# albertgassol1/vf-nerf

Hardware: AMD Instinct MI355X
Metric: rays/sec (4096-ray chunk, 128 samples/ray) + PSNR vs ref (higher is better)
Workload: dtype f16x3+f32acc

## Files before the change

### vf_nerf_amd/csrc/vfn_mlp16.hip

```cpp
#include <string.h>
#include <utility>
#include "vfn_common.h"
#include "vfn_plan.h"

typedef _Float16 half8 __attribute__((ext_vector_type(8)));
typedef _Float16 half2v __attribute__((ext_vector_type(2)));
typedef float float2v __attribute__((ext_vector_type(2)));
typedef float f32x16 __attribute__((ext_vector_type(16)));
typedef float f32x4v __attribute__((ext_vector_type(4)));

#ifndef VFN16_ASCALE
#define VFN16_ASCALE 1
#endif
#define VFN16_WSCALE 64.0f
#define VFN16_INV_WSCALE 0.015625f
#define VFN16_PACK_WSCALE (VFN16_ASCALE ? 1.0f : VFN16_WSCALE)
#define VFN16_XSCALE (VFN16_ASCALE ? VFN16_WSCALE : 1.0f)
#ifndef VFN16_SAVE_AUX
#define VFN16_SAVE_AUX 2
#endif
#ifndef VFN16_HANDOVER_NUM
#define VFN16_HANDOVER_NUM 8
#endif
#ifndef VFN16_DMA_STEPS
// ... 248 lines not shown
constexpr ChunkD chunk_of(int mode, int c) {
    if (!(mode & M16_BLKIN)) {
        const int vf_layers = (mode & M16_FEAT) ? 9 : 8;
        for (int h = 0; h < vf_layers; ++h) {
            if (c < VF_TILES[h]) return {0, vf_off_kb(h) + c * chunk_kb(VF_ACT[h], VF_AUX[h]), chunk_kb(VF_ACT[h], VF_AUX[h]), VF_AUX[h]};
            c -= VF_TILES[h];
        }
        if (c == 0) return {0, vf_off_kb(9), HEAD_KB, 0};
        c -= 1;
    }
    if (mode & M16_RENDER) {
        for (int h = 0; h < 4; ++h) {
            if (c < RN_TILES[h]) return {1, rn_off_kb(h) + c * chunk_kb(RN_ACT[h], RN_AUX[h]), chunk_kb(RN_ACT[h], RN_AUX[h]), RN_AUX[h]};
            c -= RN_TILES[h];
        }
        if (c == 0) return {1, rn_off_kb(4), HEAD_KB, 0};
    }
    return {0, 0, 0, 0};
}

constexpr int rn_first_chunk(int mode) { return (mode & M16_BLKIN) ? 0 : 72; }
constexpr bool chunk_two(int mode, int c) { return (mode & M16_C2) && !(mode & M16_BLKIN) && c >= 63 && c != 71; }
constexpr bool mode_one(int mode) { return (mode & M16_P1) != 0; }
#ifndef VFN16_P1_RING
#define VFN16_P1_RING 5
#endif
#define VFN16_P1_SLOT_KB 20
constexpr int ring_of(int mode) { return mode_one(mode) ? VFN16_P1_RING : 3; }
constexpr int slot_u4(int mode) { return mode_one(mode) ? VFN16_P1_SLOT_KB * 64 : VFN16_MAX_CHUNK_KB * 64; }
constexpr int slot_base(int mode, int c) { return (c % ring_of(mode)) * slot_u4(mode); }
static_assert(VFN16_P1_RING * VFN16_P1_SLOT_KB <= 3 * VFN16_MAX_CHUNK_KB, "the single-product ring must fit into the split modes' ring");
constexpr int stores_of(int mode, int c) { return (c == 0 || ((mode & M16_RENDER) && c == rn_first_chunk(mode))) ? 0 : 4; }
constexpr int young_ops(int mode, int c) {
    const int ring = ring_of(mode);
    int n = 0;
    for (int k = (c - ring + 2 > 0 ? c - ring + 2 : 0); k < c; ++k) n += stores_of(mode, k);
    for (int j = 2; j <= ring - 2; ++j)
        if (c + j >= ring - 1 && chunk_of(mode, c + j).kb > 0) n += (((chunk_of(mode, c + j).kb - 1) / 2 + 1) / VFN16_WAVES);
    return n;
}

struct Mlp16Args {
    const uint4* vf_w;
    const uint4* rn_w;
    const float* points;
    const float* ray_dirs;
    float* out_vec;
    float* out_colors;
    long long n_points;
    int dirs_div;
    int vf_multires, rn_multires;
    uint32_t vf_bytes, rn_bytes;
    float* saved;
    float* save_aux_vf;
// ... 17 lines not shown
#define VFN16_RANGE_TRACK 2
#endif

struct X16 { half8 hi[16]; half8 lo[16]; };
struct A16 { half8 hi[3]; half8 lo[3]; };

struct Pipe16 {
    uint4* lds;
    __amdgpu_buffer_rsrc_t vf_w;
    __amdgpu_buffer_rsrc_t rn_w;
    float* saved;
    long long slot_floats;
    uint32_t slot_bytes;
    uint32_t save_voff;
    uint32_t save_voff16;
    uint32_t feat_voff;
    uint32_t st_tile, st_q;
    int save16;
    uint32_t* masks;
    uint32_t mask_bytes;
    uint32_t mask_voff;
    uint4* blk_out;
    uint32_t blk_bytes, blk_voff;
};

struct Carry16 {
    f32x16 pend;
    f32x16 bias;
    half8 fh0, fl0;
    uint32_t lm[4];
    unsigned long long sat;
};

template <int N, typename F, int... I>
__device__ __forceinline__ void static_for_impl(F&& f, std::integer_sequence<int, I...>) { (f(std::integral_constant<int, I>{}), ...); }
template <int N, typename F>
__device__ __forceinline__ void static_for(F&& f) { static_for_impl<N>(f, std::make_integer_sequence<int, N>{}); }

__device__ __forceinline__ void split2(float a, float b, _Float16& h0, _Float16& h1, _Float16& l0, _Float16& l1) {
    const float2v v = {a, b};
    const half2v hi = __builtin_convertvector(v, half2v);
    h0 = hi[0]; h1 = hi[1];
    const uint32_t hp = __builtin_bit_cast(uint32_t, hi);
    float r0, r1;
    asm("v_fma_mix_f32 %0, %1, -1.0, %2 op_sel_hi:[1,0,0]" : "=v"(r0) : "v"(hp), "v"(a));
    asm("v_fma_mix_f32 %0, %1, -1.0, %2 op_sel:[1,0,0] op_sel_hi:[1,0,0]" : "=v"(r1) : "v"(hp), "v"(b));
    const float2v r = {r0, r1};
    const half2v lo = __builtin_convertvector(r, half2v);
    l0 = lo[0]; l1 = lo[1];
}

__device__ __forceinline__ float tanh_exp(float v) { return 1.0f - 2.0f / (1.0f + expf(2.0f * v)); }

template <int NET, int OFF_KB, int LDS_U4>
__device__ __forceinline__ void dma_piece(const Pipe16& p, int blk, int lane, int dst_blk = -1) {
    __builtin_amdgcn_raw_ptr_buffer_load_lds(NET ? p.rn_w : p.vf_w, (lds_void*)(p.lds + LDS_U4 + (dst_blk < 0 ? blk : dst_blk) * 64), 16,
                                             lane * 16, (OFF_KB + blk) * 1024, 0, 0);
}
template <int MODE, int C>
__device__ __forceinline__ void dma_chunk(const Pipe16& p, int wave, int lane) {
    constexpr ChunkD d = chunk_of(MODE, C);
    if constexpr (mode_one(MODE)) {
        constexpr int NKB = (d.kb - 1) / 2;
#pragma unroll
        for (int i = 0; i * VFN16_WAVES < NKB + 1; ++i)
            if (wave + VFN16_WAVES * i < NKB + 1) dma_piece<d.net, d.off_kb, slot_base(MODE, C)>(p, 2 * (wave + VFN16_WAVES * i), lane, wave + VFN16_WAVES * i);
    } else {
#pragma unroll
    for (int i = 0; i * VFN16_WAVES < d.kb; ++i)
        if (wave + VFN16_WAVES * i < d.kb) dma_piece<d.net, d.off_kb, slot_base(MODE, C)>(p, wave + VFN16_WAVES * i, lane);
    }
}

template <int MODE, int C>
__device__ __forceinline__ void prefetch_chunk(Carry16& cy, const Pipe16& p, int lane) {
    constexpr ChunkD d = chunk_of(MODE, C);
    const uint4* cb = p.lds + slot_base(MODE, C);
    const f32x4v* bb = reinterpret_cast<const f32x4v*>(cb + (mode_one(MODE) ? (d.kb - 1) / 2 : d.kb - 1) * 64) + (lane >> 5) * 4;
    const f32x4v b0 = bb[0], b1 = bb[1], b2 = bb[2], b3 = bb[3];
#pragma unroll
    for (int q = 0; q < 4; ++q) { cy.bias[q] = b0[q]; cy.bias[4 + q] = b1[q]; cy.bias[8 + q] = b2[q]; cy.bias[12 + q] = b3[q]; }
    cy.fh0 = __builtin_bit_cast(half8, cb[0 * 64 + lane]);
    if (!chunk_two(MODE, C) && !mode_one(MODE)) cy.fl0 = __builtin_bit_cast(half8, cb[1 * 64 + lane]);
}

template <int EPI, bool KEEP, bool LO = true>
__device__ __forceinline__ void epi_pair(f32x16& pend, unsigned long long& sat, int pr, half8& hi, half8& lo, int j) {
    float v0 = pend[2 * pr], v1 = pend[2 * pr + 1];
#if VFN16_RANGE_TRACK == 1
    if (EPI == EPI_RELU) sat |= __builtin_amdgcn_ballot_w64(fmaxf(v0, v1) >= VFN16_CLAMP);
#endif
    if (!VFN16_ASCALE || EPI != EPI_RELU) { v0 *= VFN16_INV_WSCALE; v1 *= VFN16_INV_WSCALE; }
    if (EPI == EPI_RELU) {
        v0 = fminf(fmaxf(v0, 0.f), VFN16_CLAMP); v1 = fminf(fmaxf(v1, 0.f), VFN16_CLAMP);
    }
    else { v0 = tanh_exp(v0) * VFN16_XSCALE; v1 = tanh_exp(v1) * VFN16_XSCALE; }
    if constexpr (LO) {
        _Float16 h0, h1, l0, l1;
        split2(v0, v1, h0, h1, l0, l1);
        hi[j] = h0; hi[j + 1] = h1; lo[j] = l0; lo[j + 1] = l1;
// ... 85 lines not shown

template <int MODE, int C0, int ACT, int AUX, int NCH, int EPI, int PEPI, int PKB, int SLOT = -1, int PSLOT = -1, bool BLK = false,
          bool PBLK = false>
__device__ __forceinline__ void layer16(const X16& xin, const A16& aux, X16& xout, X16& xpend, Carry16& cy, float (&head)[3],
                                       const Pipe16& p, int wave, int lane) {
    constexpr int NKB = ACT + AUX;
    constexpr int E = NKB / 2 > 0 ? NKB / 2 : 1;
    constexpr int H = NKB * VFN16_HANDOVER_NUM / 16 > 0 ? NKB * VFN16_HANDOVER_NUM / 16 : 1;
    constexpr int PMAX = (VFN16_MAX_CHUNK_KB + VFN16_WAVES - 1) / VFN16_WAVES;
    constexpr int DSPAN = NKB - H > 0 ? NKB - H : 1;
    constexpr int DSTEPS = DSPAN < VFN16_DMA_STEPS ? DSPAN : VFN16_DMA_STEPS;
    static_assert(PEPI < 0 || PKB >= E, "the pending tile must be complete before it is read");
    constexpr bool TRAIN = (MODE & M16_TRAIN) != 0;
    constexpr bool LATE = TRAIN && VFN16_LATE_STORES;
    constexpr int DEND = LATE ? (NKB - 4 > H + 1 ? NKB - 4 : (H + 1 < NKB ? H + 1 : NKB - 1)) : 0;
    constexpr int SBEG = LATE ? DEND : H;
    constexpr int SSTEPS = LATE ? (NKB - DEND > 0 ? NKB - DEND : 1) : (DSPAN < 4 ? DSPAN : 4);
    constexpr int DST = LATE ? (DEND - H > 0 ? DEND - H : 1) : DSTEPS;
    constexpr int MPARTS = (LATE && E <= H) ? (DEND - H >= 4 ? 4 : (DEND - H >= 2 ? 2 : (DEND - H >= 1 ? 1 : 0))) : 0;
    static_for<NCH>([&](auto ich) {
        constexpr int ch = decltype(ich)::value;
        constexpr int C = C0 + ch;
        constexpr int RING = ring_of(MODE);
        constexpr ChunkD dcur = chunk_of(MODE, C), dnext = chunk_of(MODE, C + 1), ddma = chunk_of(MODE, C + RING - 1);
        static_assert(dcur.kb == 2 * NKB + 1, "layer shape and chunk table disagree");
        constexpr bool P1 = mode_one(MODE);
        constexpr bool W2 = chunk_two(MODE, C);
        constexpr bool D2 = chunk_two(MODE, C + RING - 1) || P1;
        constexpr int DNKB = (ddma.kb - 1) / 2;
        constexpr int DPIECES = P1 ? DNKB + 1 : (D2 ? DNKB + ddma.aux + 1 : ddma.kb);
        auto piece_blk = [&](int idx) -> int {
            if (P1) return idx < DNKB ? 2 * idx : 2 * DNKB;
            if (!D2) return idx;
            if (ddma.aux == 0) return 2 * idx;
            return idx < DNKB ? 2 * idx : (idx < DNKB + ddma.aux ? 2 * (idx - ddma.aux) + 1 : 2 * DNKB);
        };
        constexpr int PM = D2 ? (DPIECES + VFN16_WAVES - 1) / VFN16_WAVES : PMAX;
        const uint4* cb = p.lds + slot_base(MODE, C);
        constexpr int FB = P1 ? 1 : 2;
        f32x16 acc = cy.bias;
        half8 fh[VFN16_FDEPTH], fl[VFN16_FDEPTH];
        fh[0] = cy.fh0;
        if (!P1 && (!W2 || ACT == 0)) fl[0] = cy.fl0;
        if (VFN16_FDEPTH == 3 && NKB > 1) {
            fh[1] = __builtin_bit_cast(half8, cb[FB * 64 + lane]);
            if (!W2 && !P1) fl[1] = __builtin_bit_cast(half8, cb[3 * 64 + lane]);
        }
        half8 ehi[2], elo[2];
        [[maybe_unused]] unsigned mbits = 0;
#pragma unroll
        for (int st = 0; st < NKB; ++st) {
            constexpr int AHEAD = VFN16_FDEPTH - 1;
            if (st + AHEAD < NKB) {
                fh[(st + AHEAD) % VFN16_FDEPTH] = __builtin_bit_cast(half8, cb[(FB * (st + AHEAD)) * 64 + lane]);
                if (!P1 && (!W2 || st + AHEAD >= ACT)) fl[(st + AHEAD) % VFN16_FDEPTH] = __builtin_bit_cast(half8, cb[(2 * (st + AHEAD) + 1) * 64 + lane]);
            }
            const half8 a_hi = fh[st % VFN16_FDEPTH];
            const half8 x_hi = st < ACT ? xin.hi[st < ACT ? st : 0] : aux.hi[st >= ACT ? st - ACT : 0];
            const half8 x_lo = st < ACT ? xin.lo[st < ACT ? st : 0] : aux.lo[st >= ACT ? st - ACT : 0];
            acc = __builtin_amdgcn_mfma_f32_32x32x16_f16(a_hi, x_hi, acc, 0, 0, 0);
#ifndef ABL_P1
// ... 14 lines not shown
                    if (ch > 0) epi_pair<EPI, TRAIN, !P1>(cy.pend, cy.sat, pr, ehi[sblk], elo[sblk], j);
                    else epi_pair<(PEPI >= 0 ? PEPI : 0), TRAIN, !P1>(cy.pend, cy.sat, pr, ehi[sblk], elo[sblk], j);
                    if ((pr & 3) == 3) {
                        asm volatile("" : "+a"(ehi[sblk]));
                        if constexpr (!P1) asm volatile("" : "+a"(elo[sblk]));
                        if (ch > 0) { xout.hi[2 * (ch > 0 ? ch - 1 : 0) + sblk] = ehi[sblk]; if constexpr (!P1) xout.lo[2 * (ch > 0 ? ch - 1 : 0) + sblk] = elo[sblk]; }
                        else { xpend.hi[PKB + sblk] = ehi[sblk]; if constexpr (!P1) xpend.lo[PKB + sblk] = elo[sblk]; }
                    }
                }
#ifndef VFN16_NOGROUPS
                if constexpr (!P1) {
                __builtin_amdgcn_sched_group_barrier(0x100, W2 ? 1 : 2, 0);
                __builtin_amdgcn_sched_group_barrier(0x008, 1, 0);
                __builtin_amdgcn_sched_group_barrier(0x002, W2 ? VFN16_EPI_PER_MFMA2 : VFN16_EPI_PER_MFMA, 0);
                __builtin_amdgcn_sched_group_barrier(0x008, 1, 0);
                __builtin_amdgcn_sched_group_barrier(0x002, W2 ? VFN16_EPI_PER_MFMA2 : VFN16_EPI_PER_MFMA, 0);
                if (!W2) {
                    __builtin_amdgcn_sched_group_barrier(0x008, 1, 0);
                    __builtin_amdgcn_sched_group_barrier(0x002, VFN16_EPI_PER_MFMA, 0);
                }
                }
#endif
            }
            if (st == H - 1 && dnext.kb > 0) {
#ifndef ABL_NOSYNC
#ifdef ABL_LOOSE_WAIT
                if ((MODE & M16_TRAIN) != 0) asm volatile("s_waitcnt vmcnt(4)" ::: "memory");
                else
#endif
                if constexpr (P1 && LATE) {
                    constexpr int young = young_ops(MODE, C);
                    static_assert(young < 64, "vmcnt is a 6-bit field");
                    if constexpr (young == 0) asm volatile("s_waitcnt vmcnt(0)" ::: "memory");
                    else asm volatile("s_waitcnt vmcnt(%0)" :: "n"(young) : "memory");
                } else
                if (LATE && C > 0 && (ch == 0 || ch > 1 || PEPI >= 0)) asm volatile("s_waitcnt vmcnt(4)" ::: "memory");
                else asm volatile("s_waitcnt vmcnt(0)" ::: "memory");
                __builtin_amdgcn_s_barrier();
#endif
            }
#ifndef ABL_NODMA
            if (st >= H && st < H + DST && ddma.kb > 0) {
#pragma unroll
                for (int i = (st - H) * PM / DST; i < (st - H + 1) * PM / DST; ++i) {
                    if (VFN16_WAVES * i + VFN16_WAVES <= DPIECES) dma_piece<ddma.net, ddma.off_kb, slot_base(MODE, C + RING - 1)>(p, piece_blk(wave + VFN16_WAVES * i), lane, P1 ? wave + VFN16_WAVES * i : -1);
                    else if (VFN16_WAVES * i < DPIECES) {
                        const int idx = min(wave + VFN16_WAVES * i, DPIECES - 1);
                        dma_piece<ddma.net, ddma.off_kb, slot_base(MODE, C + RING - 1)>(p, piece_blk(idx), lane, P1 ? idx : -1);
                    }
                }
            }
#endif
#ifndef ABL_NOMASK
            if (TRAIN && MPARTS > 0 && st >= H && st < H + MPARTS && (ch > 0 || PEPI >= 0)) {
                static_for<MPARTS>([&](auto ip) {
                    constexpr int part = decltype(ip)::value;
                    if (st - H == part) {
                        if (ch > 0) collect_mask_part<(ch > 0 ? ch - 1 : 0), EPI, part, (MPARTS > 0 ? MPARTS : 1)>(cy, mbits);
                        else collect_mask_part<PKB / 2, (PEPI >= 0 ? PEPI : 0), part, (MPARTS > 0 ? MPARTS : 1)>(cy, mbits);
                    }
                });
            }
#endif
            if (TRAIN && st >= SBEG && st < SBEG + SSTEPS && (ch > 0 || PEPI >= 0)) {
#ifndef ABL_NOMASK
                if (st == (LATE ? SBEG : VFN16_MASK_STEP(H, NKB))) {
                    if constexpr (MPARTS > 0) {
                        if (ch == 0) store_mask<(PSLOT >= 0 ? PSLOT : 0)>(p, cy);
                    } else {
                        if (ch > 0) collect_mask<(ch > 0 ? ch - 1 : 0), EPI>(cy);
                        else { collect_mask<PKB / 2, (PEPI >= 0 ? PEPI : 0)>(cy); store_mask<(PSLOT >= 0 ? PSLOT : 0)>(p, cy); }
                    }
                }
#endif
#pragma unroll
                for (int q = (st - SBEG) * 4 / SSTEPS; q < (st - SBEG + 1) * 4 / SSTEPS; ++q) {
                    if (ch > 0) save_group<(SLOT >= 0 ? SLOT : 0), (ch > 0 ? ch - 1 : 0), (MODE & M16_SF16) != 0>(p, cy.pend, q);
                    else save_group<(PSLOT >= 0 ? PSLOT : 0), PKB / 2, (MODE & M16_SF16) != 0>(p, cy.pend, q);
                }
            }
            if (st == H && ((BLK && ch > 0) || (PBLK && ch == 0))) {
                if (ch > 0) store_blocks<(ch > 0 ? ch - 1 : 0)>(p, xout);
                else store_blocks<PKB / 2>(p, xpend);
            }
            if (st == NKB - 1 && dnext.kb > 0) prefetch_chunk<MODE, (dnext.kb > 0 ? C + 1 : C)>(cy, p, lane);
#ifndef VFN16_NOSCHED
            __builtin_amdgcn_sched_barrier(0);
#endif
        }
        if (EPI == EPI_RELU || EPI == EPI_TANH) {
            cy.pend = acc;
#if VFN16_RANGE_TRACK == 2
            if (EPI == EPI_RELU) {
                float mx = fmaxf(acc[0], acc[1]);
#pragma unroll
                for (int r = 2; r < 16; r += 2) mx = fmaxf(mx, fmaxf(acc[r], acc[r + 1]));
                cy.sat |= __builtin_amdgcn_ballot_w64(mx >= VFN16_CLAMP);
            }
#endif
        } else {
#pragma unroll
            for (int c = 0; c < 3; ++c) {
                const float v = acc[c] * VFN16_INV_WSCALE;
                head[c] = (EPI == EPI_HEAD_TANH) ? tanh_exp(v) : 1.0f / (1.0f + expf(-v));
            }
        }
    });
}
// ... 91 lines not shown
    layer16<MODE, C0 + 16, 16, 0, 8, R, R, 14, 11, 10>(xb, aux, xa, xb, cy, rgb, p, wave, lane);
    layer16<MODE, C0 + 24, 16, 0, 8, R, R, 14, 12, 11>(xa, aux, xb, xa, cy, rgb, p, wave, lane);
    layer16<MODE, C0 + 32, 16, 0, 1, EPI_HEAD_SIGMOID, R, 14, -1, 12>(xb, aux, xa, xb, cy, rgb, p, wave, lane);
    const long long mo = m;
    if (in && (threadIdx.x & 32) == 0) {
        a.out_vec[mo * 3 + 0] = nrm[0]; a.out_vec[mo * 3 + 1] = nrm[1]; a.out_vec[mo * 3 + 2] = nrm[2];
        a.out_colors[mo * 3 + 0] = rgb[0]; a.out_colors[mo * 3 + 1] = rgb[1]; a.out_colors[mo * 3 + 2] = rgb[2];
    }
}

__device__ __forceinline__ void report_range(const Mlp16Args& a, unsigned long long sat, float ain) {
    if (a.status) {
        const unsigned bits = (sat != 0ull ? 1u : 0u) | (ain >= VFN16_CLAMP ? 2u : 0u);
        if (bits) atomicOr(a.status, bits);
    }
}

template <int MODE>
__global__ __launch_bounds__(256, 1) void vfn_mlp16_kernel(const Mlp16Args a) {
    __shared__ __attribute__((aligned(16))) uint4 s_ring[3 * VFN16_SLOT + 256 * 8];
    float* s_park = reinterpret_cast<float*>(s_ring + 3 * VFN16_SLOT) + threadIdx.x * 32;
    const int tid = threadIdx.x;
    const int lane = tid & 63;
    const int wave = __builtin_amdgcn_readfirstlane(tid >> 6);
    const int g = lane >> 5;
#ifdef VFN16_STAMPS
    const unsigned long long st_t0 = __builtin_amdgcn_s_memtime(), st_r0 = __builtin_amdgcn_s_memrealtime();
#endif
    unsigned long long ck_t0 = 0ull, ck_r0 = 0ull;
    if constexpr ((MODE & M16_RENDER) != 0 && (MODE & M16_BLKIN) == 0 && (MODE & M16_TRAIN) == 0) {
        if (a.clock) { ck_t0 = __builtin_amdgcn_s_memtime(); ck_r0 = __builtin_amdgcn_s_memrealtime(); }
    }
    const long long m = (long long)blockIdx.x * VFN16_PTS + wave * 32 + (lane & 31);
    long long n_live = a.n_points;
    if (a.n_dev) {
        const long long nd = (long long)*a.n_dev;
        n_live = nd < n_live ? nd : n_live;
        if ((long long)blockIdx.x * VFN16_PTS >= n_live) return;
    }
    const bool in = m < n_live;

    if constexpr ((MODE & M16_BLKIN) != 0) {
        const int dpos = in ? a.src[m] : -1;
        const bool live = dpos >= 0;
        float xr[3] = {0.f, 0.f, 0.f}, dr[3] = {0.f, 0.f, 0.f}, nrm[3] = {0.f, 0.f, 0.f};
        if (live) {
            const long long di = dpos / a.dirs_div;
#pragma unroll
            for (int c = 0; c < 3; ++c) { xr[c] = a.points[(long long)dpos * 3 + c]; dr[c] = a.ray_dirs[di * 3 + c]; nrm[c] = a.vec_in[m * 3 + c]; }
        }
        Pipe16 p;
        p.lds = s_ring;
        p.vf_w = __builtin_amdgcn_make_buffer_rsrc(const_cast<uint4*>(a.rn_w), 0, (int)a.rn_bytes, 0x00020000);
        p.rn_w = p.vf_w;
        p.saved = nullptr; p.slot_floats = 0; p.slot_bytes = 0; p.save_voff = 0; p.blk_out = nullptr; p.blk_bytes = 0; p.blk_voff = 0;
        p.masks = nullptr; p.mask_bytes = 0; p.mask_voff = 0; p.save16 = 0; p.save_voff16 = 0; p.feat_voff = 0; p.st_tile = 0; p.st_q = 0;
        dma_chunk<MODE, 0>(p, wave, lane);
        dma_chunk<MODE, 1>(p, wave, lane);
        X16 xa, xb;
        A16 aux;
        float ain_blk = 0.f;
        {
            typedef unsigned int u32x4 __attribute__((ext_vector_type(4)));
            const __amdgpu_buffer_rsrc_t rs_blk = __builtin_amdgcn_make_buffer_rsrc(
                const_cast<uint4*>(a.blk_in), 0, (int)(((a.n_points + 31) & ~31ll) * 1024), 0x00020000);
            const unsigned goff = in ? (unsigned)((m >> 5) * 32768 + lane * 16) : 0xfffffff0u;
            u32x4 q[32];
#pragma unroll
            for (int i = 0; i < 32; ++i) q[i] = __builtin_amdgcn_raw_buffer_load_b128(rs_blk, goff, i * 1024, 0);
            render_aux<MODE>(a, aux, xr, dr, nrm, -1, false, g, ain_blk);
#pragma unroll
            for (int t = 0; t < 8; ++t) {
                half8 h0 = __builtin_bit_cast(half8, q[4 * t + 0]), l0 = __builtin_bit_cast(half8, q[4 * t + 1]);
                half8 h1 = __builtin_bit_cast(half8, q[4 * t + 2]), l1 = __builtin_bit_cast(half8, q[4 * t + 3]);
                asm volatile("" : "+a"(h0)); asm volatile("" : "+a"(l0)); asm volatile("" : "+a"(h1)); asm volatile("" : "+a"(l1));
                xb.hi[2 * t] = h0; xb.lo[2 * t] = l0; xb.hi[2 * t + 1] = h1; xb.lo[2 * t + 1] = l1;
            }
        }
        asm volatile("s_waitcnt vmcnt(0)" ::: "memory");
        __builtin_amdgcn_s_barrier();
        Carry16 cy;
#pragma unroll
        for (int q = 0; q < 16; ++q) cy.pend[q] = 0.f;
        cy.lm[0] = 0; cy.lm[1] = 0; cy.lm[2] = 0; cy.lm[3] = 0; cy.sat = 0ull;
        prefetch_chunk<MODE, 0>(cy, p, lane);
#ifdef VFN16_STAMPS
        const unsigned long long st_t1 = __builtin_amdgcn_s_memtime();
#endif
        render_tail<MODE>(a, p, cy, xa, xb, aux, nrm, live ? (long long)dpos : -1, live, wave, lane);
        report_range(a, cy.sat, ain_blk);
#ifdef VFN16_STAMPS
        if (threadIdx.x == 0 && live) {
            const unsigned long long t2 = __builtin_amdgcn_s_memtime(), r2 = __builtin_amdgcn_s_memrealtime();
            a.out_colors[(long long)dpos * 3 + 0] = (float)(st_t1 - st_t0); a.out_colors[(long long)dpos * 3 + 1] = (float)(t2 - st_t0);
            a.out_colors[(long long)dpos * 3 + 2] = (float)(r2 - st_r0);
        }
#endif
    } else {
    float x[3] = {0.f, 0.f, 0.f};
    if (in) { x[0] = a.points[m * 3 + 0]; x[1] = a.points[m * 3 + 1]; x[2] = a.points[m * 3 + 2]; }
    float d[3] = {0.f, 0.f, 0.f};
    int out_row = -1;
    if ((MODE & M16_RENDER) && in) {
        const long long di = m / a.dirs_div;
        d[0] = a.ray_dirs[di * 3 + 0]; d[1] = a.ray_dirs[di * 3 + 1]; d[2] = a.ray_dirs[di * 3 + 2];
        if (a.out_index) out_row = a.out_index[m];
    }
    asm volatile("s_waitcnt vmcnt(0)" ::: "memory");
    if (MODE & M16_RENDER) {
        s_park[0] = x[0]; s_park[1] = x[1]; s_park[2] = x[2];
        s_park[4] = d[0]; s_park[5] = d[1]; s_park[6] = d[2];
    }

    Pipe16 p;
    p.lds = s_ring;
    p.vf_w = __builtin_amdgcn_make_buffer_rsrc(const_cast<uint4*>(a.vf_w), 0, (int)a.vf_bytes, 0x00020000);
    p.rn_w = __builtin_amdgcn_make_buffer_rsrc(const_cast<uint4*>((MODE & M16_RENDER) ? a.rn_w : a.vf_w), 0,
                                               (int)((MODE & M16_RENDER) ? a.rn_bytes : a.vf_bytes), 0x00020000);
    const bool frag = (a.save_f16 & 2) != 0;
    const long long mw = m + a.ws_first;
    p.slot_floats = frag ? ((a.ws_points + 31) >> 5) * 8192 : a.ws_points * 256;
    p.saved = a.saved + a.ws_first * 256;
    {
        const long long left = p.slot_floats * 4 - a.ws_first * 1024;
        p.slot_bytes = (uint32_t)(left < 0x7fffffffll ? left : 0x7fffffffll);
    }
    p.save_voff = !in ? (frag ? 0xc0000000u : 0xfffffff0u) : (frag ? (uint32_t)((m >> 5) * 32768 + lane * 16) : (uint32_t)(m * 1024 + g * 16));
    p.save_voff16 = !in ? (frag ? 0xc0000000u : 0xfffffff0u) : (frag ? (uint32_t)((m >> 5) * 32768 + lane * 8) : (uint32_t)(m * 1024 + g * 8));
    p.feat_voff = in ? (uint32_t)(m * 1024 + g * 16) : 0xfffffff0u;
    p.st_tile = frag ? 4096u : 128u; p.st_q = frag ? 1024u : 32u;
    p.masks = a.save_masks; p.mask_bytes = (uint32_t)(a.ws_points * 32); p.mask_voff = in ? (uint32_t)((2 * mw + g) * 16) : 0xfffffff0u;
    p.save16 = a.save_f16 & 1;
    p.blk_out = a.blk_out; p.blk_bytes = (uint32_t)(((a.n_points + 31) & ~31ll) * 1024);
    p.blk_voff = (uint32_t)((m >> 5) * 32768 + lane * 16);
    dma_chunk<MODE, 0>(p, wave, lane);
    dma_chunk<MODE, 1>(p, wave, lane);
    if constexpr (mode_one(MODE)) static_for<VFN16_P1_RING - 3>([&](auto ic) { dma_chunk<MODE, 2 + decltype(ic)::value>(p, wave, lane); });
#ifdef ABL_NODMA
    dma_chunk<MODE, 9>(p, wave, lane);
    dma_chunk<MODE, 10>(p, wave, lane);
    dma_chunk<MODE, 11>(p, wave, lane);
#endif

    const int vf_multires = a.vf_multires;
    A16 aux;
    float ain = 0.f;
    {
        float sn[18], cs[18];
        encode_sincos(x, vf_multires, g, sn, cs);
        build_aux(aux, g, [&](int k) { return enc_value(x, sn, cs, vf_multires, k); }, ain);
        if ((MODE & M16_TRAIN) && in) save_aux(a.save_aux_vf, mw, g, [&](int k) { return enc_value(x, sn, cs, vf_multires, k); });
        half8* pk = reinterpret_cast<half8*>(s_park + 8);
#pragma unroll
        for (int q = 0; q < 3; ++q) { pk[2 * q] = aux.hi[q]; pk[2 * q + 1] = aux.lo[q]; }
    }
    asm volatile("s_waitcnt vmcnt(0)" ::: "memory");
    __builtin_amdgcn_s_barrier();
    Carry16 cy;
#pragma unroll
    for (int q = 0; q < 16; ++q) cy.pend[q] = 0.f;
    cy.lm[0] = 0; cy.lm[1] = 0; cy.lm[2] = 0; cy.lm[3] = 0; cy.sat = 0ull;
    prefetch_chunk<MODE, 0>(cy, p, lane);

    X16 xa, xb;
    float vec[3] = {0.f, 0.f, 0.f};
#ifdef VFN16_STAMPS
    const unsigned long long st_t1 = __builtin_amdgcn_s_memtime();
#endif
    constexpr int R = EPI_RELU, T = EPI_TANH, NONE = -1;
    layer16<MODE, 0, 0, 3, 8, R, NONE, 0, 0, -1>(xa, aux, xb, xb, cy, vec, p, wave, lane);
    layer16<MODE, 8, 16, 0, 8, R, R, 14, 1, 0>(xb, aux, xa, xb, cy, vec, p, wave, lane);
    layer16<MODE, 16, 16, 0, 8, R, R, 14, 2, 1>(xa, aux, xb, xa, cy, vec, p, wave, lane);
    layer16<MODE, 24, 16, 0, 7, R, R, 14, 3, 2>(xb, aux, xa, xb, cy, vec, p, wave, lane);
    { A16 ax; load_aux(ax, s_park); layer16<MODE, 31, 14, 3, 8, R, R, 12, 4, 3>(xa, ax, xb, xa, cy, vec, p, wave, lane); }
    layer16<MODE, 39, 16, 0, 8, R, R, 14, 5, 4>(xb, aux, xa, xb, cy, vec, p, wave, lane);
    layer16<MODE, 47, 16, 0, 8, R, R, 14, 6, 5>(xa, aux, xb, xa, cy, vec, p, wave, lane);
    layer16<MODE, 55, 16, 0, 8, R, R, 14, 7, 6>(xb, aux, xa, xb, cy, vec, p, wave, lane);
    if constexpr (!(MODE & M16_FEAT)) {
        layer16<MODE, 63, 16, 0, 1, EPI_HEAD_TANH, R, 14, -1, 7>(xa, aux, xb, xa, cy, vec, p, wave, lane);
        if (in && g == 0) { a.out_vec[m * 3 + 0] = vec[0]; a.out_vec[m * 3 + 1] = vec[1]; a.out_vec[m * 3 + 2] = vec[2]; }
        report_range(a, cy.sat, ain);
    } else {
    constexpr bool BO = (MODE & M16_BLKOUT) != 0;
    layer16<MODE, 63, 16, 0, 8, T, R, 14, 8, 7, BO, false>(xa, aux, xb, xa, cy, vec, p, wave, lane);
    layer16<MODE, 71, 16, 0, 1, EPI_HEAD_TANH, T, 14, -1, 8, false, BO>(xa, aux, xb, xb, cy, vec, p, wave, lane);
    if constexpr (!(MODE & M16_RENDER)) {
        if (in && g == 0) { a.out_vec[m * 3 + 0] = vec[0]; a.out_vec[m * 3 + 1] = vec[1]; a.out_vec[m * 3 + 2] = vec[2]; }
        report_range(a, cy.sat, ain);
#ifdef VFN16_STAMPS
        if (threadIdx.x == 0) {
            const unsigned long long t2 = __builtin_amdgcn_s_memtime(), r2 = __builtin_amdgcn_s_memrealtime();
            a.out_vec[m * 3 + 0] = (float)(st_t1 - st_t0); a.out_vec[m * 3 + 1] = (float)(t2 - st_t0); a.out_vec[m * 3 + 2] = (float)(r2 - st_r0);
        }
#endif
    } else {
    float nrm[3];
#pragma unroll
    for (int c = 0; c < 3; ++c) nrm[c] = __shfl(vec[c], lane & 31, 64);
    const float xr[3] = {s_park[0], s_park[1], s_park[2]};
    const float dr[3] = {s_park[4], s_park[5], s_park[6]};
    A16 raux;
    render_aux<MODE>(a, raux, xr, dr, nrm, (MODE & M16_TRAIN) ? mw : m, in, g, ain);
    render_tail<MODE>(a, p, cy, xa, xb, raux, nrm, a.out_index ? (long long)out_row : m, a.out_index ? out_row >= 0 : in, wave, lane);
    report_range(a, cy.sat, ain);
    if constexpr ((MODE & M16_TRAIN) == 0) {
        if (a.clock && threadIdx.x == 0 && (long long)blockIdx.x < a.clock_slots) {
            const unsigned long long t1 = __builtin_amdgcn_s_memtime(), r1 = __builtin_amdgcn_s_memrealtime();
            a.clock[2 * blockIdx.x] = t1 - ck_t0; a.clock[2 * blockIdx.x + 1] = r1 - ck_r0;
        }
    }
    const long long mo = (long long)blockIdx.x * VFN16_PTS + (threadIdx.x >> 6) * 32 + (threadIdx.x & 31);
    (void)mo;
#ifdef VFN16_STAMPS
    if (threadIdx.x == 0) {
        const unsigned long long t1 = __builtin_amdgcn_s_memtime(), r1 = __builtin_amdgcn_s_memrealtime();
        a.out_colors[mo * 3 + 0] = (float)(t1 - st_t0); a.out_colors[mo * 3 + 1] = (float)(r1 - st_r0);
    }
#endif
    }
    }
    }
}

int check_vf16(const Plan16& vf, const char* what) {
    bool ok = vf.feat_layer == 1 && vf.n_hidden == 9 && (int)vf.head_off_kb == vf_off_kb(9);
    for (int h = 0; ok && h < 9; ++h)
        ok = vf.act16[h] == VF_ACT[h] && vf.aux16[h] == VF_AUX[h] && vf.n_tiles[h] == VF_TILES[h] && (int)vf.off_kb[h] == vf_off_kb(h);
    if (!ok) { vfn_set_error("%s: the f16x3 kernels are specialised for the shipped vector-field network shape", what); return VFN_ERR_UNSUPPORTED; }
    return VFN_OK;
}
int check_rn16(const Plan16& rn, const char* what) {
    bool ok = rn.n_hidden == 4 && (int)rn.head_off_kb == rn_off_kb(4);
    for (int h = 0; ok && h < 4; ++h)
        ok = rn.act16[h] == RN_ACT[h] && rn.aux16[h] == RN_AUX[h] && rn.n_tiles[h] == RN_TILES[h] && (int)rn.off_kb[h] == rn_off_kb(h);
    if (!ok) { vfn_set_error("%s: the f16x3 kernels are specialised for the shipped rendering network shape", what); return VFN_ERR_UNSUPPORTED; }
    return VFN_OK;
}

}

static int check_kind16(int net_kind, const Plan16& p, const char* what) {
    return net_kind == VFN_NET_VF ? check_vf16(p, what) : check_rn16(p, what);
// ... 22 lines not shown
    : old_status(t_status_word), old_clock(t_clock_probe), old_slots(t_clock_slots) {
    if (status_word) t_status_word = status_word;
    if (clock_stamps && clock_slots > 0) { t_clock_probe = reinterpret_cast<unsigned long long*>(clock_stamps); t_clock_slots = clock_slots; }
}
VfnReportScope::~VfnReportScope() { t_status_word = old_status; t_clock_probe = old_clock; t_clock_slots = old_slots; }

extern "C" int vfn_vf_mlp16_fwd(const vfn_net_geom* geom, const void* packed16, const float* points, int64_t n_points,
                                 float* out_vec, void* stream) {
    Mlp16Args a = {};
    VfnNetPlan p32; Plan16 vf;
    int rc = make_plan16(VFN_NET_VF, geom, &p32, &vf, "vfn_vf_mlp16_fwd");
    if (rc != VFN_OK) return rc;
    rc = check_vf16(vf, "vfn_vf_mlp16_fwd");
    if (rc != VFN_OK) return rc;
    if (n_points <= 0) return VFN_OK;
    VFN_REQUIRE(packed16 && points && out_vec, "vfn_vf_mlp16_fwd: NULL argument");
    a.vf_w = (const uint4*)packed16; a.points = points; a.out_vec = out_vec; a.n_points = n_points; a.dirs_div = 1;
    a.vf_multires = vf.multires; a.vf_bytes = vf.total_kb * 1024u;
    a.status = t_status_word;
    a.clock = t_clock_probe; a.clock_slots = t_clock_slots;
    const long long blocks = (n_points + VFN16_PTS - 1) / VFN16_PTS;
    hipLaunchKernelGGL(vfn_mlp16_kernel<M16_VF_VEC>, dim3((unsigned)blocks), dim3(256), 0, (hipStream_t)stream, a);
    return vfn_check_launch("vfn_vf_mlp16_fwd");
}

static int launch_fused16(const char* what, const vfn_net_geom* vf_geom, const void* vf_packed16, const vfn_net_geom* rn_geom,
                          const void* rn_packed16, const float* points, const float* ray_dirs, int64_t n_points,
                          int32_t samples_per_ray, const int32_t* out_index, bool scatter, int32_t colour_products, float* normals,
                          float* colors, void* stream, const int32_t* n_dev = nullptr) {
    Mlp16Args a = {};
    a.n_dev = n_dev;
    VfnNetPlan p32; Plan16 vf, rn;
    VFN_REQUIRE(vf_geom && rn_geom, "%s: NULL argument", what);
    int rc = make_plan16(VFN_NET_VF, vf_geom, &p32, &vf, what);
    if (rc != VFN_OK) return rc;
    rc = make_plan16(VFN_NET_RENDER, rn_geom, &p32, &rn, what);
    if (rc != VFN_OK) return rc;
    rc = check_vf16(vf, what);
    if (rc != VFN_OK) return rc;
    rc = check_rn16(rn, what);
    if (rc != VFN_OK) return rc;
    VFN_REQUIRE(vf_geom->feature_dims == VFN_HIDDEN && rn_geom->feature_dims == VFN_HIDDEN, "%s: both nets need feature_dims == %d", what, VFN_HIDDEN);
    VFN_REQUIRE(colour_products == 2 || colour_products == 3, "%s: colour_products must be 2 or 3 (got %d)", what, colour_products);
    if (n_points <= 0) return VFN_OK;
    VFN_REQUIRE(vf_packed16 && rn_packed16 && points && ray_dirs && normals && colors && (out_index || !scatter), "%s: NULL argument", what);
    VFN_REQUIRE(samples_per_ray > 0, "%s: samples_per_ray must be > 0", what);
    a.vf_w = (const uint4*)vf_packed16; a.rn_w = (const uint4*)rn_packed16; a.points = points; a.ray_dirs = ray_dirs;
    a.out_vec = normals; a.out_colors = colors; a.out_index = out_index; a.n_points = n_points; a.dirs_div = samples_per_ray;
    a.vf_multires = vf.multires; a.rn_multires = rn.multires; a.vf_bytes = vf.total_kb * 1024u; a.rn_bytes = rn.total_kb * 1024u;
    a.status = t_status_word;
    a.clock = t_clock_probe; a.clock_slots = t_clock_slots;
    const long long blocks = (n_points + VFN16_PTS - 1) / VFN16_PTS;
    if (colour_products == 2) hipLaunchKernelGGL(vfn_mlp16_kernel<M16_FUSED | M16_C2>, dim3((unsigned)blocks), dim3(256), 0, (hipStream_t)stream, a);
    else hipLaunchKernelGGL(vfn_mlp16_kernel<M16_FUSED>, dim3((unsigned)blocks), dim3(256), 0, (hipStream_t)stream, a);
    return vfn_check_launch(what);
}

extern "C" int vfn_vf_render_fused16_fwd(const vfn_net_geom* vf_geom, const void* vf_packed16, const vfn_net_geom* rn_geom,
                                          const void* rn_packed16, const float* points, const float* ray_dirs,
                                          int64_t n_points, int32_t samples_per_ray, float* normals, float* colors,
                                          void* stream) {
    return launch_fused16("vfn_vf_render_fused16_fwd", vf_geom, vf_packed16, rn_geom, rn_packed16, points, ray_dirs, n_points, samples_per_ray,
                          nullptr, false, 3, normals, colors, stream);
}

extern "C" int vfn_vf_render_fused16_scatter(const vfn_net_geom* vf_geom, const void* vf_packed16, const vfn_net_geom* rn_geom,
                                          const void* rn_packed16, const float* points, const float* ray_dirs,
                                          int64_t n_points, int32_t samples_per_ray, const int32_t* out_index, float* normals,
                                          float* colors, void* stream) {
    return launch_fused16("vfn_vf_render_fused16_scatter", vf_geom, vf_packed16, rn_geom, rn_packed16, points, ray_dirs, n_points,
                          samples_per_ray, out_index, true, 3, normals, colors, stream);
}

extern "C" int vfn_vf_render_fused16_products(const vfn_net_geom* vf_geom, const void* vf_packed16, const vfn_net_geom* rn_geom,
                                              const void* rn_packed16, const float* points, const float* ray_dirs, int64_t n_points,
// ... 157 lines not shown
```

Baseline: 1.910 million.

## Make fused VF+render kernel persistent with cross-group weight ring and input prefetch

Launches the fused inference kernel with one block per CU and loops over point groups, so the weight DMA ring wraps across groups instead of restarting per block. The first layer's chunks are laid out so their reload for the next group can be issued during the tail chunks, and the next group's points and directions are loaded early and parked in LDS. This is meant to hide the per-block weight reload and input fetch latency and the pipeline fill cost. In exchange it limits the grid to one block per CU, which may reduce occupancy and latency hiding, and it adds tricky ring-index bookkeeping.

```diff
diff --git a/vf_nerf_amd/csrc/vfn_mlp16.hip b/vf_nerf_amd/csrc/vfn_mlp16.hip
--- a/vf_nerf_amd/csrc/vfn_mlp16.hip
+++ b/vf_nerf_amd/csrc/vfn_mlp16.hip
@@ -1,4 +1,5 @@
 #include <string.h>
+#include <atomic>
 #include <utility>
 #include "vfn_common.h"
 #include "vfn_plan.h"
@@ -294,6 +295,12 @@
 constexpr int rn_first_chunk(int mode) { return (mode & M16_BLKIN) ? 0 : 72; }
 constexpr bool chunk_two(int mode, int c) { return (mode & M16_C2) && !(mode & M16_BLKIN) && c >= 63 && c != 71; }
 constexpr bool mode_one(int mode) { return (mode & M16_P1) != 0; }
+constexpr int FUSED_CHUNKS = 105;
+constexpr bool persistent16(int mode) { return (mode & ~M16_C2) == M16_FUSED; }
+constexpr int chunk_wrap(int mode, int c) { return persistent16(mode) && c >= FUSED_CHUNKS ? c - FUSED_CHUNKS : c; }
+static_assert(FUSED_CHUNKS % 3 == 0 && chunk_of(M16_FUSED, FUSED_CHUNKS - 1).kb > 0 && chunk_of(M16_FUSED, FUSED_CHUNKS).kb == 0,
+              "the persistent ring needs a chunk count that is a multiple of its three slots");
+constexpr int NEXT_LOAD_CHUNK = 72 + 8;
 #ifndef VFN16_P1_RING
 #define VFN16_P1_RING 5
 #endif
@@ -302,6 +309,28 @@
 constexpr int slot_u4(int mode) { return mode_one(mode) ? VFN16_P1_SLOT_KB * 64 : VFN16_MAX_CHUNK_KB * 64; }
 constexpr int slot_base(int mode, int c) { return (c % ring_of(mode)) * slot_u4(mode); }
 static_assert(VFN16_P1_RING * VFN16_P1_SLOT_KB <= 3 * VFN16_MAX_CHUNK_KB, "the single-product ring must fit into the split modes' ring");
+constexpr int L0_HANDOVER2 = 5;
+constexpr int lds_base(int mode, int c) {
+    if (!persistent16(mode)) return slot_base(mode, c);
+    const int w = chunk_wrap(mode, c);
+    return w < 8 ? (w / 4) * slot_u4(mode) + (w % 4) * 7 * 64 : ((w - 6) % 3) * slot_u4(mode);
+}
+constexpr bool has_handover(int mode, int c) { return !persistent16(mode) || c == 0 || c == L0_HANDOVER2 || c >= 8; }
+constexpr ChunkD dma_of(int mode, int c) {
+    if (!persistent16(mode)) return chunk_of(mode, c + ring_of(mode) - 1);
+    if (c == 0) return chunk_of(mode, 8);
+    if (c == L0_HANDOVER2) return chunk_of(mode, 9);
+    if (c < 8) return {0, 0, 0, 0};
+    if (c == FUSED_CHUNKS - 2) return {0, 0, 28, 3};
+    if (c == FUSED_CHUNKS - 1) return {0, 28, 28, 3};
+    return chunk_of(mode, c + 2);
+}
+constexpr int dma_chunk_index(int mode, int c) {
+    if (!persistent16(mode)) return c + ring_of(mode) - 1;
+    return c == 0 ? 8 : c == L0_HANDOVER2 ? 9 : c == FUSED_CHUNKS - 2 ? 0 : c == FUSED_CHUNKS - 1 ? 4 : c + 2;
+}
+static_assert(chunk_of(M16_FUSED, 3).off_kb == 21 && chunk_of(M16_FUSED, 7).off_kb == 49 && chunk_of(M16_FUSED, 7).kb == 7 &&
+              4 * 7 <= VFN16_MAX_CHUNK_KB && (FUSED_CHUNKS - 6) % 3 == 0, "L0's chunks as two ring units");
 constexpr int stores_of(int mode, int c) { return (c == 0 || ((mode & M16_RENDER) && c == rn_first_chunk(mode))) ? 0 : 4; }
 constexpr int young_ops(int mode, int c) {
     const int ring = ring_of(mode);
@@ -365,6 +394,8 @@
     uint32_t mask_voff;
     uint4* blk_out;
     uint32_t blk_bytes, blk_voff;
+    const Mlp16Args* args;
+    float* park;
 };
 
 struct Carry16 {
@@ -373,7 +404,25 @@
     half8 fh0, fl0;
     uint32_t lm[4];
     unsigned long long sat;
+    long long nx_m, nx_live;
+    float nx_x[3], nx_d[3];
+    int nx_row;
 };
+
+__device__ __forceinline__ void next_load(const Mlp16Args& a, Carry16& cy) {
+    const long long m = cy.nx_m < cy.nx_live ? cy.nx_m : cy.nx_live - 1;
+    cy.nx_x[0] = a.points[m * 3 + 0]; cy.nx_x[1] = a.points[m * 3 + 1]; cy.nx_x[2] = a.points[m * 3 + 2];
+    const long long di = m / a.dirs_div;
+    cy.nx_d[0] = a.ray_dirs[di * 3 + 0]; cy.nx_d[1] = a.ray_dirs[di * 3 + 1]; cy.nx_d[2] = a.ray_dirs[di * 3 + 2];
+    cy.nx_row = -1;
+    if (a.out_index) cy.nx_row = a.out_index[m];
+}
+__device__ __forceinline__ void next_park(float* park, const Carry16& cy) {
+    const bool in = cy.nx_m < cy.nx_live;
+    park[0] = in ? cy.nx_x[0] : 0.f; park[1] = in ? cy.nx_x[1] : 0.f; park[2] = in ? cy.nx_x[2] : 0.f;
+    park[3] = __builtin_bit_cast(float, in ? cy.nx_row : -1);
+    park[4] = in ? cy.nx_d[0] : 0.f; park[5] = in ? cy.nx_d[1] : 0.f; park[6] = in ? cy.nx_d[2] : 0.f;
+}
 
 template <int N, typename F, int... I>
 __device__ __forceinline__ void static_for_impl(F&& f, std::integer_sequence<int, I...>) { (f(std::integral_constant<int, I>{}), ...); }
@@ -415,10 +464,17 @@
     }
 }
 
+template <int NET, int OFF_KB, int KB, int LDS_U4>
+__device__ __forceinline__ void dma_span(const Pipe16& p, int wave, int lane) {
+#pragma unroll
+    for (int i = 0; i * VFN16_WAVES < KB; ++i)
+        if (wave + VFN16_WAVES * i < KB) dma_piece<NET, OFF_KB, LDS_U4>(p, wave + VFN16_WAVES * i, lane);
+}
+
 template <int MODE, int C>
 __device__ __forceinline__ void prefetch_chunk(Carry16& cy, const Pipe16& p, int lane) {
     constexpr ChunkD d = chunk_of(MODE, C);
-    const uint4* cb = p.lds + slot_base(MODE, C);
+    const uint4* cb = p.lds + lds_base(MODE, C);
     const f32x4v* bb = reinterpret_cast<const f32x4v*>(cb + (mode_one(MODE) ? (d.kb - 1) / 2 : d.kb - 1) * 64) + (lane >> 5) * 4;
     const f32x4v b0 = bb[0], b1 = bb[1], b2 = bb[2], b3 = bb[3];
 #pragma unroll
@@ -550,11 +606,13 @@
         constexpr int ch = decltype(ich)::value;
         constexpr int C = C0 + ch;
         constexpr int RING = ring_of(MODE);
-        constexpr ChunkD dcur = chunk_of(MODE, C), dnext = chunk_of(MODE, C + 1), ddma = chunk_of(MODE, C + RING - 1);
+        constexpr int CN = chunk_wrap(MODE, C + 1), CD = dma_chunk_index(MODE, C);
+        constexpr ChunkD dcur = chunk_of(MODE, C), dnext = chunk_of(MODE, CN), ddma = dma_of(MODE, C);
+        constexpr int DBASE = lds_base(MODE, CD);
         static_assert(dcur.kb == 2 * NKB + 1, "layer shape and chunk table disagree");
         constexpr bool P1 = mode_one(MODE);
         constexpr bool W2 = chunk_two(MODE, C);
-        constexpr bool D2 = chunk_two(MODE, C + RING - 1) || P1;
+        constexpr bool D2 = chunk_two(MODE, CD) || P1;
         constexpr int DNKB = (ddma.kb - 1) / 2;
         constexpr int DPIECES = P1 ? DNKB + 1 : (D2 ? DNKB + ddma.aux + 1 : ddma.kb);
         auto piece_blk = [&](int idx) -> int {
@@ -564,7 +622,7 @@
             return idx < DNKB ? 2 * idx : (idx < DNKB + ddma.aux ? 2 * (idx - ddma.aux) + 1 : 2 * DNKB);
         };
         constexpr int PM = D2 ? (DPIECES + VFN16_WAVES - 1) / VFN16_WAVES : PMAX;
-        const uint4* cb = p.lds + slot_base(MODE, C);
+        const uint4* cb = p.lds + lds_base(MODE, C);
         constexpr int FB = P1 ? 1 : 2;
         f32x16 acc = cy.bias;
         half8 fh[VFN16_FDEPTH], fl[VFN16_FDEPTH];
@@ -625,7 +683,7 @@
                 }
 #endif
             }
-            if (st == H - 1 && dnext.kb > 0) {
+            if (st == H - 1 && dnext.kb > 0 && has_handover(MODE, C)) {
 #ifndef ABL_NOSYNC
 #ifdef ABL_LOOSE_WAIT
                 if ((MODE & M16_TRAIN) != 0) asm volatile("s_waitcnt vmcnt(4)" ::: "memory");
@@ -641,15 +699,16 @@
                 else asm volatile("s_waitcnt vmcnt(0)" ::: "memory");
                 __builtin_amdgcn_s_barrier();
 #endif
+                if constexpr (persistent16(MODE)) { if (C == NEXT_LOAD_CHUNK + 1) next_park(p.park, cy); }
             }
 #ifndef ABL_NODMA
             if (st >= H && st < H + DST && ddma.kb > 0) {
 #pragma unroll
                 for (int i = (st - H) * PM / DST; i < (st - H + 1) * PM / DST; ++i) {
-                    if (VFN16_WAVES * i + VFN16_WAVES <= DPIECES) dma_piece<ddma.net, ddma.off_kb, slot_base(MODE, C + RING - 1)>(p, piece_blk(wave + VFN16_WAVES * i), lane, P1 ? wave + VFN16_WAVES * i : -1);
+                    if (VFN16_WAVES * i + VFN16_WAVES <= DPIECES) dma_piece<ddma.net, ddma.off_kb, DBASE>(p, piece_blk(wave + VFN16_WAVES * i), lane, P1 ? wave + VFN16_WAVES * i : -1);
                     else if (VFN16_WAVES * i < DPIECES) {
                         const int idx = min(wave + VFN16_WAVES * i, DPIECES - 1);
-                        dma_piece<ddma.net, ddma.off_kb, slot_base(MODE, C + RING - 1)>(p, piece_blk(idx), lane, P1 ? idx : -1);
+                        dma_piece<ddma.net, ddma.off_kb, DBASE>(p, piece_blk(idx), lane, P1 ? idx : -1);
                     }
                 }
             }
@@ -686,7 +745,8 @@
                 if (ch > 0) store_blocks<(ch > 0 ? ch - 1 : 0)>(p, xout);
                 else store_blocks<PKB / 2>(p, xpend);
             }
-            if (st == NKB - 1 && dnext.kb > 0) prefetch_chunk<MODE, (dnext.kb > 0 ? C + 1 : C)>(cy, p, lane);
+            if constexpr (persistent16(MODE)) { if (C == NEXT_LOAD_CHUNK && st == H) next_load(*p.args, cy); }
+            if (st == NKB - 1 && dnext.kb > 0) prefetch_chunk<MODE, (dnext.kb > 0 ? CN : C)>(cy, p, lane);
 #ifndef VFN16_NOSCHED
             __builtin_amdgcn_sched_barrier(0);
 #endif
@@ -824,10 +884,11 @@
     float* s_park = reinterpret_cast<float*>(s_ring + 3 * VFN16_SLOT) + threadIdx.x * 32;
     const int tid = threadIdx.x;
     const int lane = tid & 63;
-    const int wave = __builtin_amdgcn_readfirstlane(tid >> 6);
+    const int wave_wg = __builtin_amdgcn_readfirstlane(tid >> 6);
+    const int wave = wave_wg;
     const int g = lane >> 5;
 #ifdef VFN16_STAMPS
-    const unsigned long long st_t0 = __builtin_amdgcn_s_memtime(), st_r0 = __builtin_amdgcn_s_memrealtime();
+    unsigned long long st_t0 = __builtin_amdgcn_s_memtime(), st_r0 = __builtin_amdgcn_s_memrealtime();
 #endif
     unsigned long long ck_t0 = 0ull, ck_r0 = 0ull;
     if constexpr ((MODE & M16_RENDER) != 0 && (MODE & M16_BLKIN) == 0 && (MODE & M16_TRAIN) == 0) {
@@ -857,6 +918,7 @@
         p.rn_w = p.vf_w;
         p.saved = nullptr; p.slot_floats = 0; p.slot_bytes = 0; p.save_voff = 0; p.blk_out = nullptr; p.blk_bytes = 0; p.blk_voff = 0;
         p.masks = nullptr; p.mask_bytes = 0; p.mask_voff = 0; p.save16 = 0; p.save_voff16 = 0; p.feat_voff = 0; p.st_tile = 0; p.st_q = 0;
+        p.args = &a; p.park = s_park;
         dma_chunk<MODE, 0>(p, wave, lane);
         dma_chunk<MODE, 1>(p, wave, lane);
         X16 xa, xb;
@@ -899,6 +961,8 @@
         }
 #endif
     } else {
+    constexpr bool PERSIST = persistent16(MODE);
+    static_assert(!PERSIST || (MODE & (M16_TRAIN | M16_BLKOUT | M16_BLKIN | M16_P1)) == 0, "persistent launches: fused inference only");
     float x[3] = {0.f, 0.f, 0.f};
     if (in) { x[0] = a.points[m * 3 + 0]; x[1] = a.points[m * 3 + 1]; x[2] = a.points[m * 3 + 2]; }
     float d[3] = {0.f, 0.f, 0.f};
@@ -912,6 +976,7 @@
     if (MODE & M16_RENDER) {
         s_park[0] = x[0]; s_park[1] = x[1]; s_park[2] = x[2];
         s_park[4] = d[0]; s_park[5] = d[1]; s_park[6] = d[2];
+        if constexpr (PERSIST) s_park[3] = __builtin_bit_cast(float, out_row);
     }
 
     Pipe16 p;
@@ -935,8 +1000,14 @@
     p.save16 = a.save_f16 & 1;
     p.blk_out = a.blk_out; p.blk_bytes = (uint32_t)(((a.n_points + 31) & ~31ll) * 1024);
     p.blk_voff = (uint32_t)((m >> 5) * 32768 + lane * 16);
+    p.args = &a; p.park = s_park;
+    if constexpr (PERSIST) {
+        dma_span<0, 0, 28, lds_base(MODE, 0)>(p, wave, lane);
+        dma_span<0, 28, 28, lds_base(MODE, 4)>(p, wave, lane);
+    } else {
     dma_chunk<MODE, 0>(p, wave, lane);
     dma_chunk<MODE, 1>(p, wave, lane);
+    }
     if constexpr (mode_one(MODE)) static_for<VFN16_P1_RING - 3>([&](auto ic) { dma_chunk<MODE, 2 + decltype(ic)::value>(p, wave, lane); });
 #ifdef ABL_NODMA
     dma_chunk<MODE, 9>(p, wave, lane);
@@ -945,8 +1016,32 @@
 #endif
 
     const int vf_multires = a.vf_multires;
+    float ain = 0.f;
+    Carry16 cy;
+#pragma unroll
+    for (int q = 0; q < 16; ++q) cy.pend[q] = 0.f;
+    cy.lm[0] = 0; cy.lm[1] = 0; cy.lm[2] = 0; cy.lm[3] = 0; cy.sat = 0ull;
+    cy.nx_m = 0; cy.nx_live = n_live; cy.nx_row = -1;
+#pragma unroll
+    for (int c = 0; c < 3; ++c) { cy.nx_x[c] = 0.f; cy.nx_d[c] = 0.f; }
+    long long grp = blockIdx.x;
+    for (;;) {
+    long long mg = m;
+    bool ing = in;
+    int wave = wave_wg;
+    if constexpr (PERSIST) {
+        asm volatile("" : "+s"(wave));
+        if (a.clock) { ck_t0 = __builtin_amdgcn_s_memtime(); ck_r0 = __builtin_amdgcn_s_memrealtime(); }
+#ifdef VFN16_STAMPS
+        st_t0 = __builtin_amdgcn_s_memtime(); st_r0 = __builtin_amdgcn_s_memrealtime();
+#endif
+        mg = grp * VFN16_PTS + wave * 32 + (lane & 31);
+        ing = mg < n_live;
+        x[0] = s_park[0]; x[1] = s_park[1]; x[2] = s_park[2];
+        out_row = __builtin_bit_cast(int, s_park[3]);
+        cy.nx_m = mg + (long long)gridDim.x * VFN16_PTS;
+    }
     A16 aux;
-    float ain = 0.f;
     {
         float sn[18], cs[18];
         encode_sincos(x, vf_multires, g, sn, cs);
@@ -956,13 +1051,11 @@
 #pragma unroll
         for (int q = 0; q < 3; ++q) { pk[2 * q] = aux.hi[q]; pk[2 * q + 1] = aux.lo[q]; }
     }
-    asm volatile("s_waitcnt vmcnt(0)" ::: "memory");
-    __builtin_amdgcn_s_barrier();
-    Carry16 cy;
-#pragma unroll
-    for (int q = 0; q < 16; ++q) cy.pend[q] = 0.f;
-    cy.lm[0] = 0; cy.lm[1] = 0; cy.lm[2] = 0; cy.lm[3] = 0; cy.sat = 0ull;
-    prefetch_chunk<MODE, 0>(cy, p, lane);
+    if (!PERSIST || grp == (long long)blockIdx.x) {
+        asm volatile("s_waitcnt vmcnt(0)" ::: "memory");
+        __builtin_amdgcn_s_barrier();
+        prefetch_chunk<MODE, 0>(cy, p, lane);
+    }
 
     X16 xa, xb;
     float vec[3] = {0.f, 0.f, 0.f};
@@ -1002,16 +1095,16 @@
     const float xr[3] = {s_park[0], s_park[1], s_park[2]};
     const float dr[3] = {s_park[4], s_park[5], s_park[6]};
     A16 raux;
-    render_aux<MODE>(a, raux, xr, dr, nrm, (MODE & M16_TRAIN) ? mw : m, in, g, ain);
-    render_tail<MODE>(a, p, cy, xa, xb, raux, nrm, a.out_index ? (long long)out_row : m, a.out_index ? out_row >= 0 : in, wave, lane);
-    report_range(a, cy.sat, ain);
+    render_aux<MODE>(a, raux, xr, dr, nrm, (MODE & M16_TRAIN) ? mw : mg, ing, g, ain);
+    render_tail<MODE>(a, p, cy, xa, xb, raux, nrm, a.out_index ? (long long)out_row : mg, a.out_index ? out_row >= 0 : ing, wave, lane);
+    if constexpr (!PERSIST) report_range(a, cy.sat, ain);
     if constexpr ((MODE & M16_TRAIN) == 0) {
-        if (a.clock && threadIdx.x == 0 && (long long)blockIdx.x < a.clock_slots) {
+        if (a.clock && threadIdx.x == 0 && grp < a.clock_slots) {
             const unsigned long long t1 = __builtin_amdgcn_s_memtime(), r1 = __builtin_amdgcn_s_memrealtime();
-            a.clock[2 * blockIdx.x] = t1 - ck_t0; a.clock[2 * blockIdx.x + 1] = r1 - ck_r0;
-        }
-    }
-    const long long mo = (long long)blockIdx.x * VFN16_PTS + (threadIdx.x >> 6) * 32 + (threadIdx.x & 31);
+            a.clock[2 * grp] = t1 - ck_t0; a.clock[2 * grp + 1] = r1 - ck_r0;
+        }
+    }
+    const long long mo = grp * VFN16_PTS + (threadIdx.x >> 6) * 32 + (threadIdx.x & 31);
     (void)mo;
 #ifdef VFN16_STAMPS
     if (threadIdx.x == 0) {
@@ -1020,6 +1113,16 @@
     }
 #endif
     }
+    }
+    if constexpr (!PERSIST) break;
+    else {
+        grp += gridDim.x;
+        if (grp * VFN16_PTS >= n_live) break;
+    }
+    }
+    if constexpr (PERSIST) {
+        report_range(a, cy.sat, ain);
+        asm volatile("s_waitcnt vmcnt(0)" ::: "memory");
     }
     }
 }
@@ -1088,6 +1191,17 @@
     const long long blocks = (n_points + VFN16_PTS - 1) / VFN16_PTS;
     hipLaunchKernelGGL(vfn_mlp16_kernel<M16_VF_VEC>, dim3((unsigned)blocks), dim3(256), 0, (hipStream_t)stream, a);
     return vfn_check_launch("vfn_vf_mlp16_fwd");
+}
+
+static int device_cu_count() {
+    static std::atomic<int> cached[64];
+    int dev = 0;
+    if (hipGetDevice(&dev) != hipSuccess || dev < 0) return 0;
+    if (dev < 64) { const int c = cached[dev].load(std::memory_order_relaxed); if (c > 0) return c; }
+    int cus = 0;
+    if (hipDeviceGetAttribute(&cus, hipDeviceAttributeMultiprocessorCount, dev) != hipSuccess || cus <= 0) return 0;
+    if (dev < 64) cached[dev].store(cus, std::memory_order_relaxed);
+    return cus;
 }
 
 static int launch_fused16(const char* what, const vfn_net_geom* vf_geom, const void* vf_packed16, const vfn_net_geom* rn_geom,
@@ -1116,7 +1230,10 @@
     a.vf_multires = vf.multires; a.rn_multires = rn.multires; a.vf_bytes = vf.total_kb * 1024u; a.rn_bytes = rn.total_kb * 1024u;
     a.status = t_status_word;
     a.clock = t_clock_probe; a.clock_slots = t_clock_slots;
-    const long long blocks = (n_points + VFN16_PTS - 1) / VFN16_PTS;
+    const long long groups = (n_points + VFN16_PTS - 1) / VFN16_PTS;
+    const int cus = device_cu_count();
+    if (cus <= 0) { vfn_set_error("%s: could not read the device's CU count", what); return VFN_ERR_LAUNCH; }
+    const long long blocks = groups < cus ? groups : cus;
     if (colour_products == 2) hipLaunchKernelGGL(vfn_mlp16_kernel<M16_FUSED | M16_C2>, dim3((unsigned)blocks), dim3(256), 0, (hipStream_t)stream, a);
     else hipLaunchKernelGGL(vfn_mlp16_kernel<M16_FUSED>, dim3((unsigned)blocks), dim3(256), 0, (hipStream_t)stream, a);
     return vfn_check_launch(what);
```

Measured after the change: 1.911 million, median of 4. No clear change (+0.1%).
